# ParBLiSS/kmerhash

Measured on AMD Instinct MI355X. Metric: kmer_inserts_plus_finds_per_sec, higher is better.
Workload: dtype u64

## Files before the change

kmerhash_amd/csrc/kh_kernels.h:

```cpp
#pragma once
#include <hip/hip_runtime.h>
#include <stdint.h>
#include "../../include/kmerhash_amd/kh_hash.h"

#define KH_LB 11
#define KH_L (1u << KH_LB)
#define KH_HS 4096u
#define KH_CHUNK_THREADS 512
#ifndef KH_PART_THREADS
#define KH_PART_THREADS 512
#define KH_PART_MAXPER 4
#endif
#ifndef KH_PART_ITEMS
#define KH_PART_ITEMS 16
#endif
#define KH_PART_TILE (KH_PART_THREADS * KH_PART_ITEMS)
#ifndef KH_PART_STAGE
#define KH_PART_STAGE 4096
#endif
#define KH_NONE 0xFFFFFFFFFFFFFFFFull
#define KH_EMPTY_KEY 0xFFFFFFFFFFFFFFFFull

enum { KHK_RH = 0, KHK_LP = 1 };
enum { KH_FLAG_PROBE_OVERFLOW = 0, KH_FLAG_REGION_OVERFLOW = 1, KH_FLAG_COUNT_OVERFLOW = 2, KH_FLAG_INTERNAL = 3, KH_FLAG_FUSE_INVALID = 4, KH_NFLAGS = 8 };
// ... 1484 lines not shown
    KhMP v; v.A = KH_MP_NEG; v.n = 0;
#pragma unroll
    for (int j = 0; j < KH_CARRY_ITEMS; ++j) {
      it[j].A = KH_MP_NEG; it[j].n = 0;
      if (c0 + j < nch) { it[j].A = sumA[c0 + j]; it[j].n = sumN[c0 + j]; }
      v = kh_mp_combine(v, it[j]);
    }
    KhMP total;
    KhMP excl = kh_block_scan_mp(v, s_wtot, &total);
    const KhMP carry = s_carry;
    KhMP run = kh_mp_combine(carry, excl);
#pragma unroll
    for (int j = 0; j < KH_CARRY_ITEMS; ++j) {
      if (c0 + j < nch) prefix_tmp[c0 + j] = run;
      run = kh_mp_combine(run, it[j]);
    }
    __syncthreads();
    if (tid == 0) s_carry = kh_mp_combine(carry, total);
    __syncthreads();
  }
  KhMP all = s_carry;
  long long end0 = all.A > all.n ? all.A : all.n;
  long long x0 = end0 - cap;
  if (x0 < 0) x0 = 0;
  for (uint32_t c = tid; c < nch; c += 1024) {
    KhMP p = prefix_tmp[c];
    long long x = x0 + p.n;
    xcarry[c] = p.A > x ? p.A : x;
  }
}

#define KH_SPILL 256
template <int KIND, int HASH>
__global__ __launch_bounds__(KH_CHUNK_THREADS) void k_chunk_place(KhRebuildParams P) {
  __shared__ uint64_t skeys[KH_L + KH_SPILL];
  __shared__ uint32_t svals[KH_L + KH_SPILL];
  __shared__ uint32_t sinfo_w[(KH_L + KH_SPILL) / 4];
  __shared__ uint32_t fill[KH_L];
  __shared__ uint32_t start[KH_L];
  __shared__ uint32_t s_emin;
  __shared__ long long s_pend;
  __shared__ KhMP s_wtot[KH_CHUNK_THREADS / 64];
  uint8_t* sinfo = reinterpret_cast<uint8_t*>(sinfo_w);
  const uint32_t tid = threadIdx.x, c = blockIdx.x;
  const uint32_t Ln = P.New.cap > KH_L ? KH_L : (uint32_t)P.New.cap;
  const uint64_t Sc = (uint64_t)c * Ln, mask_n = P.New.cap - 1;
  const uint32_t empty4 = KIND == KHK_RH ? 0u : 0x40404040u;
  for (uint32_t i = tid; i < KH_L + KH_SPILL; i += KH_CHUNK_THREADS) { skeys[i] = 0; svals[i] = 0; }
  for (uint32_t i = tid; i < (KH_L + KH_SPILL) / 4; i += KH_CHUNK_THREADS) sinfo_w[i] = empty4;
  uint32_t cb[KH_HOMES_PER_THREAD];
  KhMP v; v.A = KH_MP_NEG; v.n = 0;
#pragma unroll
  for (uint32_t j = 0; j < KH_HOMES_PER_THREAD; ++j) {
    uint32_t b = tid * KH_HOMES_PER_THREAD + j;
    cb[j] = b < Ln ? P.homecnt[Sc + b] : 0u;
    if (b < Ln) { KhMP h; h.A = (long long)b + cb[j]; h.n = cb[j]; v = kh_mp_combine(v, h); }
    fill[tid * KH_HOMES_PER_THREAD + j] = 0;
  }
  KhMP excl = kh_block_scan_mp(v, s_wtot, nullptr);
  const long long xr = P.xcarry[c] - (long long)Sc;
  long long p = excl.A > xr + excl.n ? excl.A : xr + excl.n;
#pragma unroll
  for (uint32_t j = 0; j < KH_HOMES_PER_THREAD; ++j) {
    uint32_t b = tid * KH_HOMES_PER_THREAD + j;
    if (b < Ln) {
      long long st = p > (long long)b ? p : (long long)b;
      start[b] = (uint32_t)st;
      p = st + cb[j];
    }
  }
  if (tid == KH_CHUNK_THREADS - 1) s_pend = p;
  __syncthreads();
  auto place = [&](uint64_t key, uint32_t val, uint64_t hn) {
    uint32_t b = (uint32_t)(hn - Sc);
    uint32_t r = atomicAdd(&fill[b], 1u);
    uint32_t prel = start[b] + r;
    uint32_t dist = prel - b;
    uint8_t ib = 0x00;
    if (KIND == KHK_RH) {
      if (dist > 127u) { atomicOr(&P.flags[KH_FLAG_PROBE_OVERFLOW], 1u); dist = 127u; }
      ib = (uint8_t)(0x80u | dist);
    }
    if (prel < KH_L + KH_SPILL) { skeys[prel] = key; svals[prel] = val; sinfo[prel] = ib; }
    else kh_slot_st(P.New.s + ((Sc + prel) & mask_n), key, val, ib);
  };
  kh_for_each_old<KIND, HASH>(P, c, &s_emin, place);
  kh_for_each_new<HASH>(P, c, place);
  __syncthreads();
  long long pend = s_pend;
  if (pend < (long long)Ln) pend = Ln;
  const uint32_t lo = xr > 0 ? (uint32_t)xr : 0u;
  uint32_t hi = pend < (long long)(KH_L + KH_SPILL) ? (uint32_t)pend : (KH_L + KH_SPILL);
  for (uint32_t s0 = lo + tid; s0 < hi; s0 += KH_CHUNK_THREADS) {
    kh_slot_st(P.New.s + ((Sc + s0) & mask_n), skeys[s0], svals[s0], sinfo[s0]);
  }
}

#define KH_XB 127u
#define KH_FSPILL 128u
struct KhFusedParams {
  KhSrcSet src; uint32_t PB;
  KhSlots New; KhSeed seed; int mode;
  unsigned long long* pub;
  uint64_t* ck0; uint32_t* cv0; uint16_t* homecnt0;
  uint32_t* maxidx;
  uint64_t n_total, half_max_load;
  uint64_t base_size;
  unsigned long long* est;
  uint32_t* flags;
  long long poll_limit;
  int nodup;
  KhRebuildParams R;
};

template <int KIND, int HASH, bool MERGE>
__device__ __forceinline__ uint32_t kh_stage_from_table(const KhRebuildParams& R, uint32_t c, uint64_t Sc, unsigned long long* lk,
                                                         unsigned long long* liv, uint32_t* n_staged, uint32_t* scratch) {
  const uint32_t tid = threadIdx.x;
  const uint64_t cap_o = R.Old.cap, mask_o = cap_o - 1, mask_n = R.New.cap - 1;
  if (tid == 0) *n_staged = 0;
  __syncthreads();
  if (cap_o) {
    const uint32_t nch_o = (uint32_t)(cap_o >> KH_LB);
    const uint32_t o = c & (nch_o - 1);
    const bool same = R.New.cap == cap_o;
    const uint64_t S = (uint64_t)o * KH_L;
    uint64_t len = KH_L + 128u;
    if (KIND == KHK_LP) {
      const uint64_t beyond = cap_o - KH_L;
// ... 1234 lines not shown
    if ((late >> k) & 1u) {
      const uint32_t p0 = pj[k] & 0xFFFFu, pc = (pj[k] >> 16) + xr;
      enter(kh_slot_key(w[k]), w[k].z, rank[k] >> 16, p0 > pc ? p0 : pc);
    }
  }
#pragma unroll
  for (uint32_t u = 0; u < 2; ++u) {
    if ((late >> (ROWS + u)) & 1u) {
      const uint32_t i = tid + u * KH_CHUNK_THREADS;
      const uint32_t p0 = pj[ROWS + u] & 0xFFFFu, pc = (pj[ROWS + u] >> 16) + xr;
      enter(rk[i], (uint32_t)riv[i], hbr[u], p0 > pc ? p0 : pc);
    }
  }
  __syncthreads();
  {
    const int tA = total.A > 0 ? total.A : 0;
    int pend = tA > (int)xr + (int)n_c ? tA : (int)xr + (int)n_c;
    if (pend < (int)KH_L) pend = (int)KH_L;
    if (pend > (int)(KH_L + KH_FSPILL)) pend = (int)(KH_L + KH_FSPILL);
#pragma unroll
    for (uint32_t k = 0; k < ROWS; ++k) {
      const int s0 = (int)(base + 64u * k);
      if (k < nrows && s0 >= (int)xr && s0 < pend) {
        const uint32_t ib = iinfo[s0];
        KhSlot* dst = P.New.s + ((Sc + (uint32_t)s0) & mask_n);
        if (ib == 0u) kh_slot_st(dst, 0, 0, kh_empty_info<KHK_RH>());
        else kh_slot_st(dst, ikey[s0], ival[s0], ib);
      }
    }
  }
  (void)n_old;
}

__global__ void k_fused_tail_carry(const unsigned long long* __restrict__ pub, uint32_t nch, long long* __restrict__ xcarry0,
                                   uint64_t* __restrict__ noff0 = nullptr, uint32_t* __restrict__ ncnt0 = nullptr) {
  if (threadIdx.x == 0 && blockIdx.x == 0) {
    xcarry0[0] = (long long)((pub[nch - 1] >> 32) & 0x7FFFFFFFull);
    if (noff0) { noff0[0] = 0; noff0[1] = 0; }
    if (ncnt0) ncnt0[0] = (uint32_t)pub[0];
  }
}

__global__ __launch_bounds__(1024) void k_fused_totals(const unsigned long long* __restrict__ pub, const uint32_t* __restrict__ maxidx, uint32_t nch,
                                                       unsigned long long* __restrict__ totals) {
  __shared__ unsigned long long ws[16];
  __shared__ uint32_t wm[16];
  unsigned long long sum = 0; uint32_t mx = 0;
  for (uint32_t c = blockIdx.x * 1024 + threadIdx.x; c < nch; c += gridDim.x * 1024) { sum += pub[c] & 0xFFFFFFFFull; const uint32_t v = maxidx[c]; mx = v > mx ? v : mx; }
  for (int off = 32; off > 0; off >>= 1) { sum += __shfl_down(sum, off, 64); const uint32_t o = __shfl_down(mx, off, 64); mx = o > mx ? o : mx; }
  if ((threadIdx.x & 63) == 0) { ws[threadIdx.x >> 6] = sum; wm[threadIdx.x >> 6] = mx; }
  __syncthreads();
  if (threadIdx.x == 0) {
    unsigned long long t = 0; uint32_t m = 0;
    for (int w = 0; w < 16; ++w) { t += ws[w]; m = wm[w] > m ? wm[w] : m; }
    if (t) atomicAdd(&totals[0], t);
    if (m) atomicMax(&totals[1], (unsigned long long)m);
  }
}

__global__ void k_disp_hist(const KhSlot* __restrict__ slots, uint64_t cap, unsigned long long* __restrict__ out128) {
  __shared__ uint32_t h[128];
  if (threadIdx.x < 128) h[threadIdx.x] = 0;
  __syncthreads();
  uint64_t i = (uint64_t)blockIdx.x * blockDim.x + threadIdx.x;
  uint64_t stride = (uint64_t)gridDim.x * blockDim.x;
  for (; i < cap; i += stride) { uint32_t b = slots[i].info & 0xFFu; if (b >= 0x80u) atomicAdd(&h[b & 0x7Fu], 1u); }
  __syncthreads();
  if (threadIdx.x < 128 && h[threadIdx.x]) atomicAdd(&out128[threadIdx.x], (unsigned long long)h[threadIdx.x]);
}

template <int KIND>
__global__ void k_unpack_slots(const KhSlot* __restrict__ slots, uint64_t cap, uint64_t* __restrict__ keys, uint32_t* __restrict__ vals,
                               uint8_t* __restrict__ info, uint8_t* __restrict__ flags) {
// ... 690 lines not shown
```

kmerhash_amd/csrc/kmerhash_amd.hip:

```cpp
#include "kh_kernels.h"
#include "kh_kernels_wide.h"
#include "kh_kernels_values.h"
#include "kh_kernels_index.h"
#include "kh_kernels_index_wide.h"
#include "kh_kernels_csr.h"
#include "kh_part_sizing.h"
#include "../../include/kmerhash_amd.h"

#include <string>
#include <vector>
#include <cstdio>
#include <cstring>
#include <algorithm>
#include <cmath>
#include <cstdlib>

#include <map>
#include <memory>
#include <mutex>
#include <unordered_map>

#define KH_VERSION_STR "kmerhash_amd 0.1 (gfx950)"

namespace {
// ... 24 lines not shown
      P.cached -= it->first;
      P.free_.erase(it);
      return hipSuccess;
    }
  }
  void* p = nullptr;
  hipError_t e = hipMalloc(&p, bytes);
  if (e != hipSuccess) {
    (void)hipGetLastError();
    pool_trim(dev);
    e = hipMalloc(&p, bytes);
    if (e != hipSuccess) return e;
  }
  std::lock_guard<std::mutex> g(P.m);
  P.size_of[p] = bytes;
  *out = p;
  return hipSuccess;
}
void pool_free(int dev, void* p) {
  if (!p) return;
  DevPool& P = g_pool[dev & 15];
  std::lock_guard<std::mutex> g(P.m);
  auto it = P.size_of.find(p);
  if (it == P.size_of.end()) { hipFree(p); return; }
  P.free_.insert(std::make_pair(it->second, p));
  P.cached += it->second;
}
struct HostPool { std::mutex m; std::vector<uint64_t*> pinned; std::vector<hipEvent_t> events[16]; };
HostPool g_host;
uint64_t* pinned_get() {
  { std::lock_guard<std::mutex> g(g_host.m);
    if (!g_host.pinned.empty()) { uint64_t* p = g_host.pinned.back(); g_host.pinned.pop_back(); return p; } }
  uint64_t* p = nullptr;
  if (hipHostMalloc(reinterpret_cast<void**>(&p), 64 * sizeof(uint64_t)) != hipSuccess) { (void)hipGetLastError(); return nullptr; }
  return p;
}
void pinned_put(uint64_t* p) { if (p) { std::lock_guard<std::mutex> g(g_host.m); g_host.pinned.push_back(p); } }
hipEvent_t event_get(int dev) {
  { std::lock_guard<std::mutex> g(g_host.m);
    auto& v = g_host.events[dev & 15];
    if (!v.empty()) { hipEvent_t e = v.back(); v.pop_back(); return e; } }
  hipEvent_t e = nullptr;
  hipEventCreate(&e);
  return e;
}
void event_put(int dev, hipEvent_t e) { if (e) { std::lock_guard<std::mutex> g(g_host.m); g_host.events[dev & 15].push_back(e); } }
}

namespace {

struct ProfRec { const char* name; hipEvent_t a, b; };

struct Block { char* p; size_t cap; };

}

struct SlackShared { unsigned long long* cur2; uint64_t* starts; uint32_t* ovf; uint64_t slot; };
struct SlotBuf {
  void* p; uint64_t cap;
  SlotBuf() : p(nullptr), cap(0) {}
  SlotBuf(KhSlots s) : p(s.s), cap(s.cap) {}
  SlotBuf(KwSlots s) : p(s.s), cap(s.cap) {}
};
struct kh_table {
  int kind = KHK_RH, hash = 0, device = 0;
  KhSeed seed = KhSeed{0, 0u};
  hipStream_t stream = nullptr;
  float min_lf = 0.f, max_lf = 0.f;
  uint64_t min_load = 0, max_load = 0, lsize = 0;
  uint32_t slot_bytes = sizeof(KhSlot);
  SlotBuf cur, spare;
  std::vector<Block> blocks;
  size_t blk = 0, off = 0;
  uint64_t* hpin = nullptr;
  std::string err;
  struct {
    bool active, fallback, nodup; int mode;
    bool repeatable, slack, rec12;
    SlackShared sh;
    uint64_t n_total, fed, cap_u; uint32_t PB;
    ulonglong2 *tmp, *fin;
    KhSrcSet S;
    uint64_t* stage_k; uint32_t* stage_v;
    const uint64_t* wk[KH_MAX_SRC]; const uint32_t* wv[KH_MAX_SRC]; uint64_t wn[KH_MAX_SRC]; uint32_t wsrc; uint32_t* wcnt;
  } ins = {};
  uint32_t* part_overflow = nullptr;
  double batch_vf = 1.0;
  bool batch_nodup = false;
  bool prof = false;
  std::vector<ProfRec> recs;
  std::vector<std::pair<std::string, std::pair<double, uint64_t> > > prof_acc;
};
struct kh_wtable : kh_table {};

namespace {

inline uint64_t next_pow2(uint64_t x) {
  if (x <= 1) return 1;
  return uint64_t(1) << (64 - __builtin_clzll(x - 1));
}
inline uint64_t threshold(uint64_t buckets, float lf) {
  return static_cast<uint64_t>(static_cast<float>(buckets) * lf);
}
inline uint32_t log2u(uint64_t x) { return 63u - (uint32_t)__builtin_clzll(x); }

kh_status fail(kh_table* t, kh_status s, const std::string& msg) {
  if (t) t->err = msg;
// ... 134 lines not shown
  switch (h) {                                                                        \
    case KHH_IDENTITY: { constexpr int HASH = KHH_IDENTITY; __VA_ARGS__; } break;     \
    case KHH_MURMUR3_X86: { constexpr int HASH = KHH_MURMUR3_X86; __VA_ARGS__; } break; \
    case KHH_MURMUR3_X64: { constexpr int HASH = KHH_MURMUR3_X64; __VA_ARGS__; } break; \
    default: { constexpr int HASH = KHH_FARM; __VA_ARGS__; } break;                   \
  }
#define KH_SWITCH_KIND_HASH(k, h, ...)                                                \
  if ((k) == KHK_RH) { constexpr int KIND = KHK_RH; KH_SWITCH_HASH(h, __VA_ARGS__) }  \
  else { constexpr int KIND = KHK_LP; KH_SWITCH_HASH(h, __VA_ARGS__) }

inline uint32_t grid_for(uint64_t n, uint32_t block, uint32_t maxblocks = 256 * 16) {
  uint64_t g = (n + block - 1) / block;
  if (g < 1) g = 1;
  if (g > maxblocks) g = maxblocks;
  return (uint32_t)g;
}

template <typename T>
kh_status stage_in(kh_table* t, const void* p, uint64_t n, kh_mem where, const T** out) {
  if (where == KH_MEM_DEVICE || p == nullptr) { *out = static_cast<const T*>(p); return KH_OK; }
  T* d = nullptr;
  TAKE(d, T, n);
  HIPCHK(hipMemcpyAsync(d, p, sizeof(T) * n, hipMemcpyHostToDevice, t->stream));
  *out = d;
  return KH_OK;
}

inline size_t ws_rebuild(uint64_t cap) { return size_t(cap) * 2 + (cap > KH_L ? (cap >> KH_LB) : 1) * 48 + (size_t(1) << 16); }

struct PreCount { uint16_t* homecnt; long long* sumA; long long* sumN; };

const bool g_disable_fused_rebuild = getenv("KH_DISABLE_FUSED_BUILD") != nullptr || getenv("KH_DISABLE_FUSED_REBUILD") != nullptr;

const long long g_poll_limit = getenv("KH_DEBUG_POLL_LIMIT") ? atoll(getenv("KH_DEBUG_POLL_LIMIT")) : (1ll << 23);
struct FusedRun { unsigned long long* totals; uint32_t* flags; };
const bool g_disable_lean = getenv("KH_DISABLE_LEAN_BUILD") != nullptr;
kh_status launch_fused(kh_table* t, int src, KhFusedParams& F, const KhSlots& nw, uint32_t PB_tail, const char* name, FusedRun* out) {
  const uint32_t nch = (uint32_t)(nw.cap >> KH_LB);
  char* blk; uint32_t* maxidx; uint64_t* ck0; uint32_t* cv0; uint16_t* hc0; long long* xc0; uint64_t* noff0; uint32_t* ncnt0;
  const size_t sz_pub = (size_t)nch * 8, sz_ctl = sz_pub + 256, sz_all = sz_ctl + (size_t)nch * 4;
  TAKE(blk, char, sz_all);
  maxidx = reinterpret_cast<uint32_t*>(blk + sz_ctl);
  TAKE(ck0, uint64_t, KH_DD_M); TAKE(cv0, uint32_t, KH_DD_M); TAKE(hc0, uint16_t, KH_L); TAKE(xc0, long long, 1);
  TAKE(noff0, uint64_t, 2); TAKE(ncnt0, uint32_t, 1);
  HIPCHK(hipMemsetAsync(blk, 0, sz_all, t->stream));
  F.New = nw; F.seed = t->seed;
  F.pub = reinterpret_cast<unsigned long long*>(blk);
  unsigned long long* totals = reinterpret_cast<unsigned long long*>(blk + sz_pub);
  F.maxidx = maxidx; F.ck0 = ck0; F.cv0 = cv0; F.homecnt0 = hc0;
  F.est = reinterpret_cast<unsigned long long*>(blk + sz_pub + 32);
  F.flags = reinterpret_cast<uint32_t*>(blk + sz_pub + 64);
  F.poll_limit = g_poll_limit;
  F.R.New = nw; F.R.seed = t->seed; F.R.flags = F.flags;
  { Launch L(t, name);
    const double mean_c = (double)F.n_total / (double)nch;
    const bool lean_fits = mean_c + 5.0 * std::sqrt(mean_c) < (double)KH_LEAN_M;
    if (src == 0 && F.nodup && F.src.rec12 == 1 && F.src.n == 1 && lean_fits && !g_disable_lean) { KH_SWITCH_KIND_HASH(t->kind, t->hash, hipLaunchKernelGGL((k_build_lean<KIND, HASH>), dim3(nch), dim3(KH_CHUNK_THREADS), 0, t->stream, F)); }
    else if (src == 0) { KH_SWITCH_KIND_HASH(t->kind, t->hash, hipLaunchKernelGGL((k_build_fused<KIND, HASH, 0>), dim3(nch), dim3(KH_CHUNK_THREADS), 0, t->stream, F)); }
    else if (src == 1) { KH_SWITCH_KIND_HASH(t->kind, t->hash, hipLaunchKernelGGL((k_build_fused<KIND, HASH, 1>), dim3(nch), dim3(KH_CHUNK_THREADS), 0, t->stream, F)); }
    else if (src == 3) { KH_SWITCH_HASH(t->hash, hipLaunchKernelGGL((k_build_fused<KHK_RH, HASH, 3>), dim3(nch), dim3(KH_CHUNK_THREADS), 0, t->stream, F)); }
    else if (src == 4) { KH_SWITCH_HASH(t->hash, hipLaunchKernelGGL((k_erase_stream<HASH>), dim3(nch), dim3(KH_CHUNK_THREADS), 0, t->stream, F)); }
    else if (src == 5) { KH_SWITCH_HASH(t->hash, hipLaunchKernelGGL((k_insert_stream<HASH>), dim3(nch), dim3(KH_CHUNK_THREADS), 0, t->stream, F)); }
    else { KH_SWITCH_KIND_HASH(t->kind, t->hash, hipLaunchKernelGGL((k_build_fused<KIND, HASH, 2>), dim3(nch), dim3(KH_CHUNK_THREADS), 0, t->stream, F)); } }
  { Launch L(t, "k_fused_totals");
    hipLaunchKernelGGL(k_fused_totals, dim3(std::max<uint32_t>(1u, std::min<uint32_t>(64u, nch / 1024u))), dim3(1024), 0, t->stream, F.pub, maxidx, nch, totals); }
  {
    Launch L(t, "k_fused_tail");
    hipLaunchKernelGGL(k_fused_tail_carry, dim3(1), dim3(64), 0, t->stream, F.pub, nch, xc0, noff0, ncnt0);
    KhRebuildParams T0;
    memset(&T0, 0, sizeof(T0));
    T0.Old = kNoSlots; T0.New = nw; T0.ck = ck0; T0.cv = cv0; T0.noff = noff0; T0.ncnt = ncnt0; T0.PB = PB_tail;
    T0.seed = t->seed; T0.homecnt = hc0; T0.xcarry = xc0; T0.flags = F.flags;
    KH_SWITCH_KIND_HASH(t->kind, t->hash, hipLaunchKernelGGL((k_chunk_place<KIND, HASH>), dim3(1), dim3(KH_CHUNK_THREADS), 0, t->stream, T0));
  }
  HIPCHK(hipGetLastError());
  HIPCHK(hipMemcpyAsync(t->hpin, blk + sz_pub, 128, hipMemcpyDeviceToHost, t->stream));
  t->hpin[30] = 0;
  if (t->part_overflow) HIPCHK(hipMemcpyAsync(t->hpin + 30, t->part_overflow, 4, hipMemcpyDeviceToHost, t->stream));
  HIPCHK(hipStreamSynchronize(t->stream));
  out->totals = totals; out->flags = F.flags;
  return KH_OK;
}

const char* const kProbeOverflowText = "Robin Hood probe distance would exceed 127 (7-bit info field, hashmap_robinhood.hpp:142-144,556)";
const char* const kDedupOverflowText = "internal: de-duplication set overflow";
kh_status flags_status(kh_table* t, const uint32_t* f) {
  if (f[KH_FLAG_PROBE_OVERFLOW]) return fail(t, KH_ERR_PROBE_OVERFLOW, kProbeOverflowText);
  if (f[KH_FLAG_REGION_OVERFLOW]) return fail(t, KH_ERR_PROBE_OVERFLOW, "cluster longer than one chunk (2048 slots) without an empty slot");
  if (f[KH_FLAG_COUNT_OVERFLOW]) return fail(t, KH_ERR_PROBE_OVERFLOW, "more than 65535 keys share one home bucket");
  if (f[KH_FLAG_INTERNAL]) return fail(t, KH_ERR_HIP, kDedupOverflowText);
  return KH_OK;
}

struct Narrow {
  typedef KhSlots Slots; typedef KhRebuildParams Params;
  static Slots view(const SlotBuf& b) { return narrow(b); }
  static void set_seed(Params& P, const kh_table* t) { P.seed = t->seed; }
  static void count(kh_table* t, uint32_t nch, const Params& P) {
    Launch L(t, "k_chunk_count");
    KH_SWITCH_KIND_HASH(t->kind, t->hash, hipLaunchKernelGGL((k_chunk_count<KIND, HASH>), dim3(nch), dim3(KH_CHUNK_THREADS), 0, t->stream, P));
  }
  static void place(kh_table* t, uint32_t nch, const Params& P) {
    Launch L(t, "k_chunk_place");
    KH_SWITCH_KIND_HASH(t->kind, t->hash, hipLaunchKernelGGL((k_chunk_place<KIND, HASH>), dim3(nch), dim3(KH_CHUNK_THREADS), 0, t->stream, P));
  }
};
struct Wide {
  typedef KwSlots Slots; typedef KwRebuildParams Params;
  static Slots view(const SlotBuf& b) { return wide(b); }
  static void set_seed(Params& P, const kh_table* t) { P.seed = t->seed.s; }
  static void count(kh_table* t, uint32_t nch, const Params& P) {
// ... 267 lines not shown
inline int reduce_op(int mode) { return is_reduce(mode) ? mode - INS_PLUS : 0; }
inline bool one_launch_mode(int mode) { return mode == INS_FIRST || mode == INS_UPDATE || mode == INS_PLUS; }
inline const char* apply_label(int mode) { return mode == INS_PLUS ? "k_apply_plus" : "k_apply_reduce"; }
static_assert(KH_REDUCE_MIN == KH_ROP_MIN && KH_REDUCE_MAX == KH_ROP_MAX && KH_REDUCE_OR == KH_ROP_OR && KH_REDUCE_PLUS == KH_ROP_PLUS, "kh_reduce_op is the kernels' rop");
inline bool ins_flags_ok(unsigned flags) {
  if (flags & ~(unsigned)(KH_INS_REDUCE_PLUS | KH_INS_REPEATABLE | KH_INS_REDUCE_OP_MASK)) return false;
  return (flags & KH_INS_REDUCE_PLUS) || !(flags & KH_INS_REDUCE_OP_MASK);
}
inline int ins_flags_mode(unsigned flags) {
  return (flags & KH_INS_REDUCE_PLUS) ? INS_PLUS + (int)((flags & KH_INS_REDUCE_OP_MASK) >> KH_INS_REDUCE_OP_SHIFT) : INS_FIRST;
}
const uint64_t g_max_pass = getenv("KH_MAX_PASS_RECORDS") ? std::max<uint64_t>(1024, std::min<uint64_t>(strtoull(getenv("KH_MAX_PASS_RECORDS"), nullptr, 10), 0xFFFFFFF0ull))
                                                          : (uint64_t(1) << 30);
bool g_disable_fused = getenv("KH_DISABLE_FUSED_BUILD") != nullptr;

const kh_status KH_RETRY_EXACT = static_cast<kh_status>(100);
kh_status insert_finish(kh_table* t, KhSrcSet S, uint64_t n, uint32_t PB, uint64_t cap_u, int mode, uint64_t forced_cap,
                        ulonglong2* spare, uint64_t* n_new_out, uint64_t list_cap = 0);

inline bool fused_build_applies(const kh_table* t, uint64_t cap_u, uint32_t PB) {
  return t->lsize == 0 && cap_u >= 2 * (uint64_t)KH_L && t->max_lf <= 0.9f && PB == log2u(cap_u >> KH_LB) && !g_disable_fused;
}
inline bool nodup_build_applies(const kh_table* t, uint64_t cap_u, uint32_t PB, int mode) {
  return fused_build_applies(t, cap_u, PB) && t->batch_nodup && (mode == INS_FIRST || mode == INS_PLUS) && !getenv("KH_DISABLE_NODUP");
}

kh_status insert_core(kh_table* t, const char* kbase, uint32_t kstride, const char* vbase, uint32_t vstride,
                      uint64_t n, int mode, uint64_t forced_cap, uint64_t* n_new_out) {
  *n_new_out = 0;
  if (n == 0) return KH_OK;
  const uint64_t cap_u = forced_cap ? forced_cap : capacity_after(t, t->cur.cap, t->lsize, n, n, n - 1);
  const uint32_t PB = cap_u > KH_L ? log2u(cap_u >> KH_LB) : 0u;
  if (PB > 22) return fail(t, KH_ERR_UNSUPPORTED, "batch would need more than 2^22 partitions");
  const size_t keep_blk = t->blk, keep_off = t->off;
  int first_attempt = 0;
  bool dup_heavy = false;
  double vf = 1.0;
  if (part_buffer_records(n, PB, true) != n) {
    unsigned long long* sset; uint32_t* dups;
    TAKE(sset, unsigned long long, KH_SAMPLE_SET); TAKE(dups, uint32_t, 1);
    HIPCHK(hipMemsetAsync(sset, 0, sizeof(unsigned long long) * KH_SAMPLE_SET, t->stream));
    HIPCHK(hipMemsetAsync(dups, 0, 4, t->stream));
    { Launch L(t, "k_sample_dups");
      hipLaunchKernelGGL(k_sample_dups, dim3(KH_SAMPLE_N / 256), dim3(256), 0, t->stream, kbase, kstride, n, sset, dups); }
    HIPCHK(hipMemcpyAsync(t->hpin + 31, dups, 4, hipMemcpyDeviceToHost, t->stream));
    HIPCHK(hipStreamSynchronize(t->stream));
    const uint32_t dsample = (uint32_t)t->hpin[31];
    if (dsample >= 1u) {
      dup_heavy = true;
      const double d_ub = (double)dsample + 3.0 * std::sqrt((double)dsample) + 3.0;
      const double f = 1.0 + 2.0 * (double)n * d_ub / ((double)KH_SAMPLE_N * (double)KH_SAMPLE_N);
      const double mean = (double)n / (double)(uint64_t(1) << PB);
      if (!getenv("KH_DISABLE_DUP_SLACK") && (double)slack_slot(mean, f) <= 2.0 * mean) vf = f;
      else first_attempt = 1;
    }
    t->batch_nodup = dsample == 0u;
    t->blk = keep_blk; t->off = keep_off;
  } else first_attempt = 1;
  for (int attempt = first_attempt; attempt < 2; ++attempt) {
    const bool slack = attempt == 0;
    const uint64_t m = part_buffer_records(n, PB, slack, vf);
    if (!slack && attempt == 1) { t->blk = keep_blk; t->off = keep_off; }
    const bool rec12 = slack && t->batch_nodup && nodup_build_applies(t, cap_u, PB, mode);
    const bool rec8 = !rec12 && dup_heavy && mode == INS_PLUS && vbase == nullptr && !getenv("KH_DISABLE_REC8");
    const int kind = rec12 ? 1 : rec8 ? 2 : 0;
    ulonglong2 *tmp, *fin, *spare;
    { char *a, *b; const size_t rb = kind == 1 ? sizeof(KhRec12) : kind == 2 ? sizeof(KhRec8) : sizeof(ulonglong2);
      TAKE(a, char, m * rb); TAKE(b, char, m * rb);
      tmp = reinterpret_cast<ulonglong2*>(a); fin = reinterpret_cast<ulonglong2*>(b); spare = tmp;
      if (kind == 2) { char* c; TAKE(c, char, m * 12); spare = reinterpret_cast<ulonglong2*>(c); } }
    Partitioned R;
    kh_status st = partition_batch(t, kbase, kstride, vbase, vstride, mode == INS_PLUS ? 1u : 0u, n, 0, PB, tmp, fin, R, slack, kind, nullptr, false, vf);
    if (st != KH_OK) return st;
    KhSrcSet S;
    memset(&S, 0, sizeof(S));
    S.rec[0] = R.rec; S.off[0] = R.part_off; S.n = 1; S.merged_off = R.part_off; S.slot[0] = R.slot; S.cur[0] = R.cursor;
    S.rec12 = (uint32_t)R.rec12;
    t->part_overflow = R.overflow; t->batch_vf = vf;
    st = insert_finish(t, S, n, PB, cap_u, mode, forced_cap, spare, n_new_out, m);
    t->part_overflow = nullptr; t->batch_nodup = false; t->batch_vf = 1.0;
    if (st != KH_RETRY_EXACT) return st;
  }
  return fail(t, KH_ERR_HIP, "internal: exact partition reported a slot overflow");
}

kh_status insert_finish(kh_table* t, KhSrcSet S, uint64_t n, uint32_t PB, uint64_t cap_u, int mode, uint64_t forced_cap,
                        ulonglong2* spare, uint64_t* n_new_out, uint64_t list_cap) {
  *n_new_out = 0;
  if (list_cap < n) list_cap = n;
  kh_status st = KH_OK;
  const uint32_t nparts = 1u << PB;
  struct { uint32_t nparts; } R; R.nparts = nparts;
  if (fused_build_applies(t, cap_u, PB) && one_launch_mode(mode) && S.rec12 != 2 && !(t->batch_vf >= 2.0)) {
    const uint32_t nch = (uint32_t)(cap_u >> KH_LB);
    KhSlots nw;
    st = fresh_slots(t, cap_u, nw);
    if (st != KH_OK) return st;
    KhFusedParams F;
    memset(&F, 0, sizeof(F));
    F.src = S; F.PB = PB;
    F.mode = mode == INS_PLUS ? KH_DEDUP_PLUS : KH_DEDUP_FIRST;
    F.base_size = 0;
    F.n_total = n;
    F.nodup = nodup_build_applies(t, cap_u, PB, mode) ? 1 : 0;
    F.half_max_load = (cap_u >> 1) >= t->cur.cap ? threshold(cap_u >> 1, t->max_lf) : 0;
    FusedRun run;
    { kh_status fs = launch_fused(t, 0, F, nw, PB, "k_build_fused", &run); if (fs != KH_OK) return fs; }
    if (t->part_overflow && (uint32_t)t->hpin[30]) { retire_slots(t, nw); return KH_RETRY_EXACT; }
    unsigned long long* totals = run.totals;
    const uint64_t fd = t->hpin[0];
    const uint64_t flast = (mode == INS_PLUS || S.rec12) ? n - 1 : (t->hpin[1] ? t->hpin[1] - 1 : 0);
    const uint32_t* ff = reinterpret_cast<const uint32_t*>(reinterpret_cast<const char*>(t->hpin) + 64);
    bool bad = S.rec12 && fd != n;
// ... 400 lines not shown
  HIPCHK(hipGetLastError());
  HIPCHK(hipMemcpyAsync(t->hpin, offs + ntl, 8, hipMemcpyDeviceToHost, t->stream));
  HIPCHK(hipStreamSynchronize(t->stream));
  *n_out = t->hpin[0];
  return KH_OK;
}
kh_status copy_hits_selective(kh_table* t, const uint32_t* dv, const uint8_t* df, uint64_t n, uint32_t* out_vals, uint8_t* out_found) {
  std::vector<uint32_t> hv(out_vals ? n : 0); std::vector<uint8_t> hf(n);
  if (out_vals) HIPCHK(hipMemcpyAsync(hv.data(), dv, n * 4, hipMemcpyDeviceToHost, t->stream));
  HIPCHK(hipMemcpyAsync(hf.data(), df, n, hipMemcpyDeviceToHost, t->stream));
  HIPCHK(hipStreamSynchronize(t->stream));
  for (uint64_t i = 0; i < n; ++i) { if (out_found) out_found[i] = hf[i]; if (hf[i] && out_vals) out_vals[i] = hv[i]; }
  return KH_OK;
}
kh_status copy_compacted(kh_table* t, uint64_t m, const uint64_t* ck, const uint32_t* cv, uint64_t* keys_host, uint32_t* vals_host) {
  if (m && keys_host) HIPCHK(hipMemcpyAsync(keys_host, ck, m * (t->slot_bytes / 2), hipMemcpyDeviceToHost, t->stream));
  if (m && vals_host) HIPCHK(hipMemcpyAsync(vals_host, cv, m * 4, hipMemcpyDeviceToHost, t->stream));
  HIPCHK(hipStreamSynchronize(t->stream));
  return KH_OK;
}

kh_status launch_find(kh_table* t, int out_mode, const uint64_t* q, uint64_t n, uint32_t* dvals, uint8_t* dfound, uint64_t* dkeys, uint8_t* dpairs,
                      unsigned long long** hits_dev) {
  const uint64_t ntiles = (n + KH_Q_TILE - 1) / KH_Q_TILE;
  unsigned long long* ctl;
  const size_t nctl = 2 + ((out_mode == KH_FIND_COMPACT || out_mode == KH_FIND_PAIRS) ? ntiles : 0);
  TAKE(ctl, unsigned long long, nctl);
  HIPCHK(hipMemsetAsync(ctl, 0, nctl * 8, t->stream));
  KhFindParams F;
  memset(&F, 0, sizeof(F));
  F.T = narrow(t->cur); F.q = q; F.n = n; F.seed = t->seed;
  F.out_vals = dvals; F.out_found = dfound; F.out_keys = dkeys; F.out_pairs16 = dpairs;
  F.n_found = (out_mode == KH_FIND_COUNT && !hits_dev) ? nullptr : ctl;
  F.ticket = reinterpret_cast<uint32_t*>(ctl + 1); F.tile_state = ctl + 2;
  int ncu = 256;
  hipDeviceGetAttribute(&ncu, hipDeviceAttributeMultiprocessorCount, t->device);
  const uint32_t grid = (uint32_t)std::max<uint64_t>(1, std::min<uint64_t>(ntiles, (uint64_t)ncu * 8));
  const char* name = out_mode == KH_FIND_COUNT ? "k_count" : "k_find";
  { Launch L(t, name);
#define KH_FIND_LAUNCH(OUT)                                                                                                            \
    if (t->seed.xk) { KH_SWITCH_KIND_HASH(t->kind, t->hash, hipLaunchKernelGGL((k_find<KIND, HASH, OUT, true>), dim3(grid), dim3(KH_Q_THREADS), 0, t->stream, F)); }   \
    else { KH_SWITCH_KIND_HASH(t->kind, t->hash, hipLaunchKernelGGL((k_find<KIND, HASH, OUT, false>), dim3(grid), dim3(KH_Q_THREADS), 0, t->stream, F)); }
    switch (out_mode) {
      case KH_FIND_PERQUERY: KH_FIND_LAUNCH(KH_FIND_PERQUERY) break;
      case KH_FIND_COMPACT: KH_FIND_LAUNCH(KH_FIND_COMPACT) break;
      case KH_FIND_PAIRS: KH_FIND_LAUNCH(KH_FIND_PAIRS) break;
      default: KH_FIND_LAUNCH(KH_FIND_COUNT) break;
    }
#undef KH_FIND_LAUNCH
  }
  HIPCHK(hipGetLastError());
  if (hits_dev) *hits_dev = ctl;
  return KH_OK;
}

kh_status do_find(kh_table* t, const void* keys, uint64_t n, kh_mem where, uint32_t* out_vals, uint8_t* out_found,
                  uint64_t* out_ckeys, uint32_t* out_cvals, void* out_pairs, bool compacted, uint64_t* n_found) {
  if (n_found) *n_found = 0;
  if (t->ins.active) return refuse_streaming(t);
  if (n == 0) return KH_OK;
  if (!keys) return fail(t, KH_ERR_INVALID, "null keys");
  HIPCHK(hipSetDevice(t->device));
  { kh_status ps = arena_prepare(t, n * 40 + (n / KH_Q_TILE + 8) * 8 + (size_t(1) << 20)); if (ps != KH_OK) return ps; }
  const uint64_t* q;
  kh_status st = stage_in<uint64_t>(t, keys, n, where, &q);
  if (st != KH_OK) return st;
  const bool host = where == KH_MEM_HOST;
  unsigned long long* hits_dev = nullptr;
  uint64_t hits = 0;
  if (!compacted) {
    uint32_t* dv = out_vals; uint8_t* df = out_found;
    if (host && dv) TAKE(dv, uint32_t, n);
    if (host || !df) TAKE(df, uint8_t, n);
    st = launch_find(t, KH_FIND_PERQUERY, q, n, dv, df, nullptr, nullptr, &hits_dev);
    if (st != KH_OK) return st;
    HIPCHK(hipMemcpyAsync(t->hpin, hits_dev, 8, hipMemcpyDeviceToHost, t->stream));
    if (host) { st = copy_hits_selective(t, dv, df, n, out_vals, out_found); if (st != KH_OK) return st; }
    else if (n_found) HIPCHK(hipStreamSynchronize(t->stream));
    hits = t->hpin[0];
  } else {
    uint64_t* ck = out_ckeys; uint32_t* cv = out_cvals; uint8_t* cp = static_cast<uint8_t*>(out_pairs);
    if (host) {
      if (out_pairs) TAKE(cp, uint8_t, n * 16);
      else { TAKE(ck, uint64_t, n); TAKE(cv, uint32_t, n); }
    }
    st = launch_find(t, out_pairs ? KH_FIND_PAIRS : KH_FIND_COMPACT, q, n, out_pairs ? nullptr : cv, nullptr, out_pairs ? nullptr : ck,
                     out_pairs ? cp : nullptr, &hits_dev);
    if (st != KH_OK) return st;
    HIPCHK(hipMemcpyAsync(t->hpin, hits_dev, 8, hipMemcpyDeviceToHost, t->stream));
    HIPCHK(hipStreamSynchronize(t->stream));
    hits = t->hpin[0];
    if (host && hits) {
      if (out_pairs) { HIPCHK(hipMemcpyAsync(out_pairs, cp, hits * 16, hipMemcpyDeviceToHost, t->stream)); HIPCHK(hipStreamSynchronize(t->stream)); }
      else { st = copy_compacted(t, hits, ck, cv, out_ckeys, out_cvals); if (st != KH_OK) return st; }
    }
  }
  if (n_found) *n_found = hits;
  return KH_OK;
}

kh_status erase_core(kh_table* t, const void* keys, uint64_t n, kh_mem where, uint64_t* n_erased) {
  *n_erased = 0;
  if (t->ins.active) return refuse_streaming(t);
  if (n == 0) return KH_OK;
  if (!keys) return fail(t, KH_ERR_INVALID, "null keys");
  HIPCHK(hipSetDevice(t->device));
  { kh_status ps = inplace_ok(t, n) ? arena_prepare(t, n * 8 + ws_inplace(t, n))
                                    : arena_prepare(t, n * 8 + 2 * 8 * ((slack_slot((double)n / (double)std::max<uint64_t>(1, t->cur.cap >> KH_LB)) * std::max<uint64_t>(1, t->cur.cap >> KH_LB)) + KH_PART_TILE + n) +
                                                       ws_rebuild(t->cur.cap) + (t->cur.cap > KH_L ? (t->cur.cap >> KH_LB) : 1) * 96 + (n / KH_PART_TILE + 4096) * 16 + (size_t(2) << 20));
    if (ps != KH_OK) return ps; }
  const uint64_t* q;
  kh_status st = stage_in<uint64_t>(t, keys, n, where, &q);
  if (st != KH_OK) return st;
  if (t->kind == KHK_RH && n <= KH_SMALL_N && t->lsize > 0 && !g_disable_small) {
    uint64_t ne = 0; uint32_t done = 0;
    st = small_batch(t, reinterpret_cast<const char*>(q), 8, nullptr, 0, 0, (uint32_t)n, KH_SMALL_ERASE, &ne, &done);
    if (st != KH_OK) return st;
    t->lsize -= ne;
    *n_erased = ne;
    return KH_OK;
  }
  if (inplace_ok(t, n)) {
// ... 47 lines not shown
    retire_slots(t, nw);
    t->blk = keep_blk; t->off = keep_off;
  }
  unsigned long long* cnt;
  TAKE(cnt, unsigned long long, 1);
  HIPCHK(hipMemsetAsync(cnt, 0, 8, t->stream));
  { Launch L(t, "k_erase_mark");
    KH_SWITCH_KIND_HASH(t->kind, t->hash, hipLaunchKernelGGL((k_erase_mark<KIND, HASH>), dim3(grid_for(n, KH_Q_THREADS * KH_Q_ITEMS, 2048)), dim3(KH_Q_THREADS), 0, t->stream, narrow(t->cur), q, n, t->seed, cnt)); }
  HIPCHK(hipGetLastError());
  HIPCHK(hipMemcpyAsync(t->hpin, cnt, 8, hipMemcpyDeviceToHost, t->stream));
  HIPCHK(hipStreamSynchronize(t->stream));
  const uint64_t ne = t->hpin[0];
  if (ne && t->kind == KHK_RH) {
    st = rebuild(t, t->cur.cap, nullptr, nullptr, nullptr, nullptr, 0, true, t->lsize - ne);
    if (st != KH_OK) {
      hipLaunchKernelGGL(k_clear_marks, dim3(grid_for(t->cur.cap, 256)), dim3(256), 0, t->stream, narrow(t->cur));
      hipStreamSynchronize(t->stream);
      return st;
    }
  }
  t->lsize -= ne;
  *n_erased = ne;
  return KH_OK;
}

bool valid(const kh_table* t) { return t != nullptr; }
kh_status table_init(kh_table* t, int kind, int hash, uint64_t seed, uint64_t capacity, float min_lf, float max_lf, int device) {
  t->kind = kind; t->hash = hash; t->device = device; t->seed = KhSeed{seed, 0u};
  t->min_lf = min_lf; t->max_lf = max_lf;
  const uint64_t cap = next_pow2(capacity);
  if (alloc_slots(t, cap, t->cur) != KH_OK) return KH_ERR_NOMEM;
  t->hpin = pinned_get();
  if (!t->hpin) { free_slots(t, t->cur); return KH_ERR_NOMEM; }
  if (fill_empty(t, t->cur) != KH_OK || hipStreamSynchronize(t->stream) != hipSuccess) { free_slots(t, t->cur); pinned_put(t->hpin); return KH_ERR_HIP; }
  t->min_load = threshold(cap, min_lf);
  t->max_load = threshold(cap, max_lf);
  return KH_OK;
}
void table_release(kh_table* t) {
  if (!t) return;
  hipSetDevice(t->device);
  hipStreamSynchronize(t->stream);
  for (auto& r : t->recs) { event_put(t->device, r.a); event_put(t->device, r.b); }
  free_slots(t, t->cur); free_slots(t, t->spare);
  for (auto& b : t->blocks) pool_free(t->device, b.p);
  pinned_put(t->hpin);
}

}

extern "C" {

const char* kh_version(void) { return KH_VERSION_STR; }

kh_status kh_release_cached_memory(int device) {
  if (device < 0 || device >= 16) return KH_ERR_INVALID;
  if (hipSetDevice(device) != hipSuccess) return KH_ERR_HIP;
  hipDeviceSynchronize();
  pool_trim(device);
  return KH_OK;
}

kh_status kh_create(kh_table** out, kh_kind kind, uint32_t key_bytes, uint32_t val_bytes, kh_hash hash, uint64_t seed,
                    uint64_t capacity, float min_lf, float max_lf, int device) {
  if (!out) return KH_ERR_INVALID;
  *out = nullptr;
// ... 2352 lines not shown
```

Measured before the change: 47.75 billion.

## Fuse tail kernels, write control results to mapped host memory, pre-zero fused control block

Merges the tail-carry kernel and the single-block chunk-place kernel into one launch that also writes the totals and overflow words straight into mapped, coherent pinned host memory. This drops the follow-up device-to-host memcpys. The fused-build control block is now zeroed inside the same memset as the dup-sampling buffers, which removes a separate memset. The find compact/pairs path writes its hit count directly to mapped host memory instead of copying it. This cuts launches and small copies on the latency-bound insert/find path, at the cost of zero-copy host writes and more complex arena bookkeeping.

```diff
diff --git a/kmerhash_amd/csrc/kh_kernels.h b/kmerhash_amd/csrc/kh_kernels.h
--- a/kmerhash_amd/csrc/kh_kernels.h
+++ b/kmerhash_amd/csrc/kh_kernels.h
@@ -1540,7 +1540,7 @@
 
 #define KH_SPILL 256
 template <int KIND, int HASH>
-__global__ __launch_bounds__(KH_CHUNK_THREADS) void k_chunk_place(KhRebuildParams P) {
+__device__ __forceinline__ void kh_chunk_place_wg(const KhRebuildParams& P, const uint32_t c) {
   __shared__ uint64_t skeys[KH_L + KH_SPILL];
   __shared__ uint32_t svals[KH_L + KH_SPILL];
   __shared__ uint32_t sinfo_w[(KH_L + KH_SPILL) / 4];
@@ -1550,7 +1550,7 @@
   __shared__ long long s_pend;
   __shared__ KhMP s_wtot[KH_CHUNK_THREADS / 64];
   uint8_t* sinfo = reinterpret_cast<uint8_t*>(sinfo_w);
-  const uint32_t tid = threadIdx.x, c = blockIdx.x;
+  const uint32_t tid = threadIdx.x;
   const uint32_t Ln = P.New.cap > KH_L ? KH_L : (uint32_t)P.New.cap;
   const uint64_t Sc = (uint64_t)c * Ln, mask_n = P.New.cap - 1;
   const uint32_t empty4 = KIND == KHK_RH ? 0u : 0x40404040u;
@@ -1603,6 +1603,8 @@
     kh_slot_st(P.New.s + ((Sc + s0) & mask_n), skeys[s0], svals[s0], sinfo[s0]);
   }
 }
+template <int KIND, int HASH>
+__global__ __launch_bounds__(KH_CHUNK_THREADS) void k_chunk_place(KhRebuildParams P) { kh_chunk_place_wg<KIND, HASH>(P, blockIdx.x); }
 
 #define KH_XB 127u
 #define KH_FSPILL 128u
@@ -2903,13 +2905,20 @@
   (void)n_old;
 }
 
-__global__ void k_fused_tail_carry(const unsigned long long* __restrict__ pub, uint32_t nch, long long* __restrict__ xcarry0,
-                                   uint64_t* __restrict__ noff0 = nullptr, uint32_t* __restrict__ ncnt0 = nullptr) {
-  if (threadIdx.x == 0 && blockIdx.x == 0) {
+template <int KIND, int HASH>
+__global__ __launch_bounds__(KH_CHUNK_THREADS) void k_fused_tail(KhRebuildParams P, const unsigned long long* pub, uint32_t nch, long long* xcarry0, uint64_t* noff0,
+                                                                 uint32_t* ncnt0, const unsigned long long* ctl, const uint32_t* ovf, unsigned long long* host) {
+  if (threadIdx.x == 0) {
     xcarry0[0] = (long long)((pub[nch - 1] >> 32) & 0x7FFFFFFFull);
-    if (noff0) { noff0[0] = 0; noff0[1] = 0; }
-    if (ncnt0) ncnt0[0] = (uint32_t)pub[0];
-  }
+    noff0[0] = 0; noff0[1] = 0;
+    ncnt0[0] = (uint32_t)pub[0];
+  }
+  __syncthreads();
+  kh_chunk_place_wg<KIND, HASH>(P, 0u);
+  __threadfence();
+  __syncthreads();
+  if (threadIdx.x < 16) host[threadIdx.x] = __hip_atomic_load(&ctl[threadIdx.x], __ATOMIC_RELAXED, __HIP_MEMORY_SCOPE_AGENT);
+  else if (threadIdx.x == 16) host[30] = ovf ? (unsigned long long)__hip_atomic_load(ovf, __ATOMIC_RELAXED, __HIP_MEMORY_SCOPE_AGENT) : 0ull;
 }
 
 __global__ __launch_bounds__(1024) void k_fused_totals(const unsigned long long* __restrict__ pub, const uint32_t* __restrict__ maxidx, uint32_t nch,
diff --git a/kmerhash_amd/csrc/kmerhash_amd.hip b/kmerhash_amd/csrc/kmerhash_amd.hip
--- a/kmerhash_amd/csrc/kmerhash_amd.hip
+++ b/kmerhash_amd/csrc/kmerhash_amd.hip
@@ -80,7 +80,7 @@
   { std::lock_guard<std::mutex> g(g_host.m);
     if (!g_host.pinned.empty()) { uint64_t* p = g_host.pinned.back(); g_host.pinned.pop_back(); return p; } }
   uint64_t* p = nullptr;
-  if (hipHostMalloc(reinterpret_cast<void**>(&p), 64 * sizeof(uint64_t)) != hipSuccess) { (void)hipGetLastError(); return nullptr; }
+  if (hipHostMalloc(reinterpret_cast<void**>(&p), 64 * sizeof(uint64_t), hipHostMallocMapped | hipHostMallocPortable | hipHostMallocCoherent) != hipSuccess) { (void)hipGetLastError(); return nullptr; }
   return p;
 }
 void pinned_put(uint64_t* p) { if (p) { std::lock_guard<std::mutex> g(g_host.m); g_host.pinned.push_back(p); } }
@@ -121,6 +121,8 @@
   std::vector<Block> blocks;
   size_t blk = 0, off = 0;
   uint64_t* hpin = nullptr;
+  uint64_t* hpin_dev = nullptr;
+  char* pre_ctl = nullptr; size_t pre_ctl_bytes = 0;
   std::string err;
   struct {
     bool active, fallback, nodup; int mode;
@@ -321,18 +323,21 @@
 
 const bool g_disable_fused_rebuild = getenv("KH_DISABLE_FUSED_BUILD") != nullptr || getenv("KH_DISABLE_FUSED_REBUILD") != nullptr;
 
+inline size_t fused_ctl_bytes(uint32_t nch) { return (size_t)nch * 8 + 256 + (size_t)nch * 4; }
 const long long g_poll_limit = getenv("KH_DEBUG_POLL_LIMIT") ? atoll(getenv("KH_DEBUG_POLL_LIMIT")) : (1ll << 23);
 struct FusedRun { unsigned long long* totals; uint32_t* flags; };
 const bool g_disable_lean = getenv("KH_DISABLE_LEAN_BUILD") != nullptr;
 kh_status launch_fused(kh_table* t, int src, KhFusedParams& F, const KhSlots& nw, uint32_t PB_tail, const char* name, FusedRun* out) {
   const uint32_t nch = (uint32_t)(nw.cap >> KH_LB);
   char* blk; uint32_t* maxidx; uint64_t* ck0; uint32_t* cv0; uint16_t* hc0; long long* xc0; uint64_t* noff0; uint32_t* ncnt0;
-  const size_t sz_pub = (size_t)nch * 8, sz_ctl = sz_pub + 256, sz_all = sz_ctl + (size_t)nch * 4;
-  TAKE(blk, char, sz_all);
+  const size_t sz_pub = (size_t)nch * 8, sz_ctl = sz_pub + 256, sz_all = fused_ctl_bytes(nch);
+  const bool pre_zeroed = t->pre_ctl && t->pre_ctl_bytes == sz_all;
+  if (pre_zeroed) blk = t->pre_ctl; else TAKE(blk, char, sz_all);
+  t->pre_ctl = nullptr; t->pre_ctl_bytes = 0;
   maxidx = reinterpret_cast<uint32_t*>(blk + sz_ctl);
   TAKE(ck0, uint64_t, KH_DD_M); TAKE(cv0, uint32_t, KH_DD_M); TAKE(hc0, uint16_t, KH_L); TAKE(xc0, long long, 1);
   TAKE(noff0, uint64_t, 2); TAKE(ncnt0, uint32_t, 1);
-  HIPCHK(hipMemsetAsync(blk, 0, sz_all, t->stream));
+  if (!pre_zeroed) HIPCHK(hipMemsetAsync(blk, 0, sz_all, t->stream));
   F.New = nw; F.seed = t->seed;
   F.pub = reinterpret_cast<unsigned long long*>(blk);
   unsigned long long* totals = reinterpret_cast<unsigned long long*>(blk + sz_pub);
@@ -355,17 +360,15 @@
     hipLaunchKernelGGL(k_fused_totals, dim3(std::max<uint32_t>(1u, std::min<uint32_t>(64u, nch / 1024u))), dim3(1024), 0, t->stream, F.pub, maxidx, nch, totals); }
   {
     Launch L(t, "k_fused_tail");
-    hipLaunchKernelGGL(k_fused_tail_carry, dim3(1), dim3(64), 0, t->stream, F.pub, nch, xc0, noff0, ncnt0);
     KhRebuildParams T0;
     memset(&T0, 0, sizeof(T0));
     T0.Old = kNoSlots; T0.New = nw; T0.ck = ck0; T0.cv = cv0; T0.noff = noff0; T0.ncnt = ncnt0; T0.PB = PB_tail;
     T0.seed = t->seed; T0.homecnt = hc0; T0.xcarry = xc0; T0.flags = F.flags;
-    KH_SWITCH_KIND_HASH(t->kind, t->hash, hipLaunchKernelGGL((k_chunk_place<KIND, HASH>), dim3(1), dim3(KH_CHUNK_THREADS), 0, t->stream, T0));
+    KH_SWITCH_KIND_HASH(t->kind, t->hash, hipLaunchKernelGGL((k_fused_tail<KIND, HASH>), dim3(1), dim3(KH_CHUNK_THREADS), 0, t->stream, T0, F.pub, nch, xc0, noff0, ncnt0,
+                                                             reinterpret_cast<const unsigned long long*>(blk + sz_pub), (const uint32_t*)t->part_overflow,
+                                                             reinterpret_cast<unsigned long long*>(t->hpin_dev)));
   }
   HIPCHK(hipGetLastError());
-  HIPCHK(hipMemcpyAsync(t->hpin, blk + sz_pub, 128, hipMemcpyDeviceToHost, t->stream));
-  t->hpin[30] = 0;
-  if (t->part_overflow) HIPCHK(hipMemcpyAsync(t->hpin + 30, t->part_overflow, 4, hipMemcpyDeviceToHost, t->stream));
   HIPCHK(hipStreamSynchronize(t->stream));
   out->totals = totals; out->flags = F.flags;
   return KH_OK;
@@ -699,15 +702,19 @@
   const uint64_t cap_u = forced_cap ? forced_cap : capacity_after(t, t->cur.cap, t->lsize, n, n, n - 1);
   const uint32_t PB = cap_u > KH_L ? log2u(cap_u >> KH_LB) : 0u;
   if (PB > 22) return fail(t, KH_ERR_UNSUPPORTED, "batch would need more than 2^22 partitions");
-  const size_t keep_blk = t->blk, keep_off = t->off;
+  size_t keep_blk = t->blk, keep_off = t->off;
+  struct PreCtl { kh_table* t; ~PreCtl() { t->pre_ctl = nullptr; t->pre_ctl_bytes = 0; } } pre_ctl_scope{t};
   int first_attempt = 0;
   bool dup_heavy = false;
   double vf = 1.0;
   if (part_buffer_records(n, PB, true) != n) {
-    unsigned long long* sset; uint32_t* dups;
-    TAKE(sset, unsigned long long, KH_SAMPLE_SET); TAKE(dups, uint32_t, 1);
-    HIPCHK(hipMemsetAsync(sset, 0, sizeof(unsigned long long) * KH_SAMPLE_SET, t->stream));
-    HIPCHK(hipMemsetAsync(dups, 0, 4, t->stream));
+    const size_t ctl_b = (fused_build_applies(t, cap_u, PB) && one_launch_mode(mode)) ? ((fused_ctl_bytes((uint32_t)(cap_u >> KH_LB)) + 255) & ~size_t(255)) : 0;
+    const size_t set_b = sizeof(unsigned long long) * KH_SAMPLE_SET;
+    char* zb;
+    TAKE(zb, char, ctl_b + set_b + 256);
+    unsigned long long* sset = reinterpret_cast<unsigned long long*>(zb + ctl_b); uint32_t* dups = reinterpret_cast<uint32_t*>(zb + ctl_b + set_b);
+    HIPCHK(hipMemsetAsync(zb, 0, ctl_b + set_b + 256, t->stream));
+    if (ctl_b) { keep_blk = t->blk; keep_off = t->off - (set_b + 256); t->pre_ctl = zb; t->pre_ctl_bytes = fused_ctl_bytes((uint32_t)(cap_u >> KH_LB)); }
     { Launch L(t, "k_sample_dups");
       hipLaunchKernelGGL(k_sample_dups, dim3(KH_SAMPLE_N / 256), dim3(256), 0, t->stream, kbase, kstride, n, sset, dups); }
     HIPCHK(hipMemcpyAsync(t->hpin + 31, dups, 4, hipMemcpyDeviceToHost, t->stream));
@@ -746,6 +753,7 @@
     t->part_overflow = R.overflow; t->batch_vf = vf;
     st = insert_finish(t, S, n, PB, cap_u, mode, forced_cap, spare, n_new_out, m);
     t->part_overflow = nullptr; t->batch_nodup = false; t->batch_vf = 1.0;
+    t->pre_ctl = nullptr; t->pre_ctl_bytes = 0;
     if (st != KH_RETRY_EXACT) return st;
   }
   return fail(t, KH_ERR_HIP, "internal: exact partition reported a slot overflow");
@@ -1212,6 +1220,7 @@
   F.T = narrow(t->cur); F.q = q; F.n = n; F.seed = t->seed;
   F.out_vals = dvals; F.out_found = dfound; F.out_keys = dkeys; F.out_pairs16 = dpairs;
   F.n_found = (out_mode == KH_FIND_COUNT && !hits_dev) ? nullptr : ctl;
+  if (out_mode == KH_FIND_COMPACT || out_mode == KH_FIND_PAIRS) F.n_found = reinterpret_cast<unsigned long long*>(t->hpin_dev);
   F.ticket = reinterpret_cast<uint32_t*>(ctl + 1); F.tile_state = ctl + 2;
   int ncu = 256;
   hipDeviceGetAttribute(&ncu, hipDeviceAttributeMultiprocessorCount, t->device);
@@ -1267,7 +1276,6 @@
     st = launch_find(t, out_pairs ? KH_FIND_PAIRS : KH_FIND_COMPACT, q, n, out_pairs ? nullptr : cv, nullptr, out_pairs ? nullptr : ck,
                      out_pairs ? cp : nullptr, &hits_dev);
     if (st != KH_OK) return st;
-    HIPCHK(hipMemcpyAsync(t->hpin, hits_dev, 8, hipMemcpyDeviceToHost, t->stream));
     HIPCHK(hipStreamSynchronize(t->stream));
     hits = t->hpin[0];
     if (host && hits) {
@@ -1381,6 +1389,7 @@
   if (alloc_slots(t, cap, t->cur) != KH_OK) return KH_ERR_NOMEM;
   t->hpin = pinned_get();
   if (!t->hpin) { free_slots(t, t->cur); return KH_ERR_NOMEM; }
+  if (hipHostGetDevicePointer(reinterpret_cast<void**>(&t->hpin_dev), t->hpin, 0) != hipSuccess) { (void)hipGetLastError(); free_slots(t, t->cur); pinned_put(t->hpin); return KH_ERR_HIP; }
   if (fill_empty(t, t->cur) != KH_OK || hipStreamSynchronize(t->stream) != hipSuccess) { free_slots(t, t->cur); pinned_put(t->hpin); return KH_ERR_HIP; }
   t->min_load = threshold(cap, min_lf);
   t->max_load = threshold(cap, max_lf);
```

After: 48.14 billion, median of 6. Within noise of the previous version (+0.8%).
